# bcaitech1/p4-fr-sorry-math-but-love-you

Hardware: NVIDIA B200
Metric: EfficientSATRN greedy-decode images/sec (higher is better)
Workload: dtype bf16

## Files before the change

p4-fr-sorry-math-but-love-you_b200/csrc/kernels.h:

```cpp
#pragma once
#include "common.cuh"

namespace frx {

void launch_stem_conv(const float* in, const float* w, const float* scale, const float* shift, float* out,
                      int B, int Cin, int H, int W, int OH, int OW, int Cout, cudaStream_t st);
void launch_direct_conv3x3(const float* in, const float* w, const float* scale, const float* shift, float* out, int B,
                           int Cin, int H, int W, int OH, int OW, int Cout, int stride, int pad, int act,
                           cudaStream_t st);
void launch_igemm_f32(const GemmP& p, cudaStream_t st);
void launch_dwconv_f32(const DwP& p, cudaStream_t st);
void launch_se_gate_f32(const float* x, const float* w1, const float* b1, const float* w2, const float* b2,
                        float* gate, int B, int HW, int C, int R, cudaStream_t st);
void launch_maxpool2_f32(const float* in, float* out, int B, int H, int W, int C, cudaStream_t st);
void launch_pe2d_f32(const float* x, const float* w0, const float* b0, const float* w1, const float* b1,
                     const float* peh, const float* pew, float* out, int B, int h, int w, int C,
                     cudaStream_t st);
void launch_layernorm_f32(const float* x, const float* res, const float* gamma, const float* beta, float* out,
                          int M, int C, int scramble_S, cudaStream_t st);
void launch_enc_attn_f32(const float* qkv, float* out, int B, int S, int D, int heads, cudaStream_t st);
void launch_dec_gemm_f32(const DecGemmP& p, cudaStream_t st);
void launch_dec_attn_f32(const AttnP& p, int head_dim, cudaStream_t st);
void launch_fill_i32(int* p, int v, int n, cudaStream_t st);
void launch_dec_embed_f32(const int* tok, const long long* tok64, int fixed_token, const float* emb,
// ... 6 lines not shown


void launch_dec_sift_embed(float* logits, long long ld_logits, int V, long long* tokens_out, long long ld_tok, int4* state,
                           const int* flags, const int* limit, const SiftIds& ids, int* cur_tok, const float* emb,
                           const float* pe_next, float scale, float* x, int M, int D, cudaStream_t st);
void launch_sift_state_init(int4* state, int M, int sos, cudaStream_t st);
void launch_pad_mask(const long long* text, unsigned char* mask, int B, int L, int pad_id, cudaStream_t st);

void launch_swin_patch_embed(const float* img, const float* w, const float* bias, const float* g, const float* b,
                             const float* ape, float* out, int B, int IMGS, int R, int E, cudaStream_t st);
void launch_swin_window_attn(const float* qkv, const float* bias_table, float* out, int B, int R, int C, int heads, int ws,
                             int shift, cudaStream_t st);
bool launch_swin_window_attn_mma(const float* qkv, const float* bias_table, eh_t* out, int B, int R, int C, int heads,
                                 int ws, int shift, cudaStream_t st);
void launch_swin_patch_merge(const float* x, float* out, int B, int R, int C, cudaStream_t st);

void launch_beam_init(const BeamP& p, cudaStream_t st);
void launch_beam_select(const BeamP& p, cudaStream_t st);
void launch_beam_push(const BeamP& p, cudaStream_t st);
void launch_beam_finish(const BeamP& p, cudaStream_t st);

int launch_tc_igemm(TcGemmP p, cudaStream_t st);
int launch_tc_igemm_ws(TcGemmP p, int num_sms, cudaStream_t st);
void launch_pad_conv_weights(const eh_t* in, eh_t* out, long long rows, int Cin, cudaStream_t st);
void launch_h16_to_f32(const eh_t* in, float* out, long long n, cudaStream_t st);
void launch_f32_to_h16(const float* in, eh_t* out, long long n, cudaStream_t st);
void launch_stem_conv_bf16(const float* in, const float* w, const float* scale, const float* shift,
                           eh_t* out, int B, int Cin, int H, int W, int OH, int OW, int Cout, cudaStream_t st);
void launch_dwconv_bf16(const eh_t* in, const float* w, const float* scale, const float* shift,
                        eh_t* out, int B, int H, int W, int C, int OH, int OW, int stride, int pad_t,
                        int pad_l, int act, cudaStream_t st);
void launch_se_scale_bf16(eh_t* x, const float* w1, const float* b1, const float* w2, const float* b2,
                          int B, int HW, int C, int R, cudaStream_t st);
void launch_mbconv_dw_se_bf16(const eh_t* in, const float* w, const float* scale, const float* shift,
                              eh_t* out, float* mean, float* gate, const float* w1, const float* b1,
                              const float* w2, const float* b2, int B, int H, int W, int C, int OH, int OW, int stride,
                              int pad_t, int pad_l, int R, cudaStream_t st);
void launch_layernorm_bf16out(const float* x, const float* res, const float* gamma, const float* beta,
                              eh_t* out, int M, int C, int scramble_S, cudaStream_t st);
void launch_enc_attn_bf16out(const float* qkv, eh_t* out, int B, int S, int D, int heads, cudaStream_t st);
void launch_conv3x3_c24_bf16(const eh_t* in, const void* wfrag, const float* scale, const float* shift,
                             eh_t* out, int B, int H, int W, int add_res, cudaStream_t st);
void launch_lite_conv0_pool_bf16(const float* in, const float* w, const float* scale, const float* shift, eh_t* out,
                                 int B, int Cin, int H, int W, int Cout, cudaStream_t st);
void launch_maxpool2_bf16(const eh_t* in, eh_t* out, float* out_f32, int B, int H, int W, int C, cudaStream_t st);
bool launch_enc_attn_mma_bf16(const float* qkv, eh_t* out, int B, int S, int D, int heads, cudaStream_t st);
// ... 11 lines not shown
```

p4-fr-sorry-math-but-love-you_b200/csrc/kernels_tc.cu:

```cuda
#include <cuda.h>
#include <cuda_fp16.h>
#include <cudaTypedefs.h>

#include <cstdio>
#include <cstdlib>

#include "common.cuh"
#include "kernels.h"

namespace frx {

namespace {

constexpr int TC_BM = 128;
constexpr int TC_BK = 64;
constexpr int TC_STAGES = 3;
constexpr int TC_A_BYTES = TC_BM * TC_BK * 2;

__device__ __forceinline__ uint32_t smem_u32(const void* p) { return (uint32_t)__cvta_generic_to_shared(p); }

__device__ __forceinline__ void cp_async16(uint32_t dst, const void* src, uint32_t src_bytes) {
  asm volatile("cp.async.cg.shared.global [%0], [%1], 16, %2;\n" ::"r"(dst), "l"(src), "r"(src_bytes) : "memory");
}
__device__ __forceinline__ void cp_async_commit() { asm volatile("cp.async.commit_group;\n" ::: "memory"); }
// ... 14 lines not shown
__device__ __forceinline__ void tma_load_im2col(uint32_t smem_dst, const CUtensorMap* tmap, int c, int w, int h, int n,
                                                uint16_t w_off, uint16_t h_off, uint64_t* bar) {
  asm volatile(
      "cp.async.bulk.tensor.4d.shared::cluster.global.im2col.mbarrier::complete_tx::bytes [%0], [%1, {%3, %4, %5, %6}], [%2], {%7, %8};\n"
      ::"r"(smem_dst), "l"(reinterpret_cast<uint64_t>(tmap)), "r"(smem_u32(bar)), "r"(c), "r"(w), "r"(h), "r"(n),
        "h"(w_off), "h"(h_off) : "memory");
}
__device__ __forceinline__ void mbar_arrive(uint64_t* bar) {
  asm volatile("mbarrier.arrive.shared::cta.b64 _, [%0];\n" ::"r"(smem_u32(bar)) : "memory");
}
__device__ __forceinline__ void mbar_wait(uint64_t* bar, uint32_t parity) {
  const uint32_t addr = smem_u32(bar);
  uint32_t ok = 0;
  for (int spins = 0; spins < (1 << 24); ++spins) {
    asm volatile(
        "{\n"
        ".reg .pred p;\n"
        "mbarrier.try_wait.parity.shared::cta.b64 p, [%1], %2;\n"
        "selp.u32 %0, 1, 0, p;\n"
        "}\n" : "=r"(ok) : "r"(addr), "r"(parity) : "memory");
    if (ok) return;
  }
  __trap();
}

__device__ __forceinline__ uint64_t make_smem_desc(uint32_t saddr) {
  uint64_t d = 0;
  d |= (uint64_t)((saddr >> 4) & 0x3FFF);
  d |= (uint64_t)1 << 16;
  d |= (uint64_t)(1024 >> 4) << 32;
  d |= (uint64_t)1 << 46;
  d |= (uint64_t)2 << 61;
  return d;
}

__device__ __forceinline__ uint32_t make_idesc(int bn) {
  constexpr uint32_t fmt = FRX_ENC_FP16 ? 0u : 1u;
  return (1u << 4) | (fmt << 7) | (fmt << 10) | ((uint32_t)(bn >> 3) << 17) | ((uint32_t)(TC_BM >> 4) << 24);
}

__device__ __forceinline__ void umma_f16(uint32_t tmem_d, uint64_t adesc, uint64_t bdesc, uint32_t idesc, uint32_t accumulate) {
  asm volatile(
      "{\n"
      ".reg .pred p;\n"
      "setp.ne.b32 p, %4, 0;\n"
      "tcgen05.mma.cta_group::1.kind::f16 [%0], %1, %2, %3, p;\n"
// ... 60 lines not shown
        v[i + 1] = act_fast<ACT>(fmaf(v[i + 1], s.y, h.y));
        v[i + 2] = act_fast<ACT>(fmaf(v[i + 2], s.z, h.z));
        v[i + 3] = act_fast<ACT>(fmaf(v[i + 3], s.w, h.w));
      }
    }
  } else if (shift) {
#pragma unroll
    for (int i = 0; i < 16; i += 4) {
      const float4 h = __ldg(reinterpret_cast<const float4*>(shift + nb + i));
      v[i] = act_fast<ACT>(v[i] + h.x);
      v[i + 1] = act_fast<ACT>(v[i + 1] + h.y);
      v[i + 2] = act_fast<ACT>(v[i + 2] + h.z);
      v[i + 3] = act_fast<ACT>(v[i + 3] + h.w);
    }
  } else {
#pragma unroll
    for (int i = 0; i < 16; ++i) v[i] = act_fast<ACT>(v[i]);
  }
}

}

template <bool GELU>
__device__ __forceinline__ void epilogue_store16(const TcGemmP& p, const uint32_t (&r)[16], int m, int nb) {
      float v[16];
#pragma unroll
      for (int i = 0; i < 16; ++i) v[i] = __uint_as_float(r[i]);
      const bool full = nb + 16 <= p.N;
      if (full) {
        if (p.act == ACT_SILU) epi_affine_act<ACT_SILU>(v, p.scale, p.shift, nb);
        else if (p.act == ACT_RELU) epi_affine_act<ACT_RELU>(v, p.scale, p.shift, nb);
        else if (GELU && p.act == ACT_GELU) epi_affine_act<ACT_GELU>(v, p.scale, p.shift, nb);
        else epi_affine_act<ACT_NONE>(v, p.scale, p.shift, nb);
      } else {
#pragma unroll
        for (int i = 0; i < 16; ++i) {
          const int n = nb + i;
          if (n < p.N) {
            if (p.scale) v[i] = v[i] * __ldg(p.scale + n) + __ldg(p.shift + n);
            else if (p.shift) v[i] += __ldg(p.shift + n);
            v[i] = act_apply(v[i], p.act);
          }
        }
      }
      if (p.res) {
        if (p.res_f32) {
          const float* rp = reinterpret_cast<const float*>(p.res) + (size_t)m * p.ldr + nb;
          if (full) {
#pragma unroll
            for (int i = 0; i < 16; i += 4) {
              const float4 rr = __ldg(reinterpret_cast<const float4*>(rp + i));
              v[i] += rr.x; v[i + 1] += rr.y; v[i + 2] += rr.z; v[i + 3] += rr.w;
            }
          } else {
            for (int i = 0; i < 16; ++i)
              if (nb + i < p.N) v[i] += __ldg(rp + i);
          }
        } else {
          const eh_t* rp = reinterpret_cast<const eh_t*>(p.res) + (size_t)m * p.ldr + nb;
          if (full) {
            const uint4 r0 = __ldg(reinterpret_cast<const uint4*>(rp)), r1 = __ldg(reinterpret_cast<const uint4*>(rp + 8));
            const uint32_t rw[8] = {r0.x, r0.y, r0.z, r0.w, r1.x, r1.y, r1.z, r1.w};
#pragma unroll
            for (int i = 0; i < 8; ++i) {
              const float2 rf = eh2_unpack(rw[i]);
              v[2 * i] += rf.x;
              v[2 * i + 1] += rf.y;
            }
          } else {
            for (int i = 0; i < 16; ++i)
              if (nb + i < p.N) v[i] += eh_to_float(rp[i]);
          }
        }
      }
      if (p.out_f32) {
        float* cp = reinterpret_cast<float*>(p.C) + (size_t)m * p.ldc + nb;
        if (full && (p.ldc & 7) == 0 && (reinterpret_cast<uintptr_t>(p.C) & 31) == 0) {
#pragma unroll
          for (int i = 0; i < 16; i += 8)
            asm volatile("st.global.v8.f32 [%0], {%1, %2, %3, %4, %5, %6, %7, %8};\n" ::"l"(cp + i), "f"(v[i]), "f"(v[i + 1]),
                         "f"(v[i + 2]), "f"(v[i + 3]), "f"(v[i + 4]), "f"(v[i + 5]), "f"(v[i + 6]), "f"(v[i + 7]) : "memory");
        } else if (full && (p.ldc & 3) == 0) {
#pragma unroll
          for (int i = 0; i < 16; i += 4) *reinterpret_cast<float4*>(cp + i) = make_float4(v[i], v[i + 1], v[i + 2], v[i + 3]);
        } else {
// ... 160 lines not shown
      const int nb = n0 + cc * 16;
      if (m_ok && nb < p.N) epilogue_store16<false>(p, r, m, nb);
    }
  }
  tc_fence_before();
  __syncthreads();
  if (warp == 0) {
    asm volatile("tcgen05.dealloc.cta_group::1.sync.aligned.b32 %0, %1;\n" ::"r"(tmem), "n"(NCOLS) : "memory");
  }
}


constexpr int WS_STAGES = 4;
constexpr int WS_LAG = 2;
constexpr int WS_PROD_WARPS = 8;
constexpr int WS_EPI_WARPS = 8;
constexpr int WS_MMA_WARP = WS_PROD_WARPS + WS_EPI_WARPS;
constexpr int WS_TMA_WARP = WS_MMA_WARP + 1;
constexpr int WS_THREADS = (WS_TMA_WARP + 1) * 32;
constexpr int WS_PROD_THREADS = WS_PROD_WARPS * 32;
constexpr int WS_ROWS_PER_PASS = WS_PROD_THREADS / 8;
constexpr int WS_A_PASSES = TC_BM / WS_ROWS_PER_PASS;

template <int NCOLS, bool GELU>
__global__ void __launch_bounds__(WS_THREADS, NCOLS >= 256 ? 1 : 2) tc_igemm_ws_kernel(const TcGemmP p, const __grid_constant__ CUtensorMap tmA,
                                                                  const __grid_constant__ CUtensorMap tmW) {
  extern __shared__ unsigned char dyn_smem[];
  __shared__ __align__(8) uint64_t full_bar[WS_STAGES], empty_bar[WS_STAGES], acc_full[2], acc_empty[2];
  __shared__ uint32_t tmem_base_s;

  const int tid = threadIdx.x, warp = tid >> 5, lane = tid & 31;
  const int BN = p.BN;
  const uint32_t stage_bytes = TC_A_BYTES + (uint32_t)BN * (TC_BK * 2);
  const uint32_t smem0 = (smem_u32(dyn_smem) + 1023u) & ~1023u;
  const int KB = p.im2col ? p.KW * p.KW : (p.K + TC_BK - 1) / TC_BK;
  const int tiles_n = (p.N + BN - 1) / BN;
  const int tiles_m = (p.M + TC_BM - 1) / TC_BM;
  const int num_tiles = tiles_m * tiles_n;
  const bool gather = p.conv && !p.im2col;

  if (warp == WS_MMA_WARP) {
    asm volatile("tcgen05.alloc.cta_group::1.sync.aligned.shared::cta.b32 [%0], %1;\n" ::"r"(smem_u32(&tmem_base_s)), "n"(NCOLS) : "memory");
    asm volatile("tcgen05.relinquish_alloc_permit.cta_group::1.sync.aligned;\n" ::: "memory");
  }
  if (tid == 0) {
#pragma unroll
    for (int s = 0; s < WS_STAGES; ++s) { mbar_init(&full_bar[s], (gather ? WS_PROD_THREADS : 0) + 1); mbar_init(&empty_bar[s], 1); }
    mbar_init(&acc_full[0], 1); mbar_init(&acc_full[1], 1);
    const int epi_threads = (WS_EPI_WARPS + (gather ? 0 : WS_PROD_WARPS)) * 32;
    mbar_init(&acc_empty[0], epi_threads); mbar_init(&acc_empty[1], epi_threads);
    asm volatile("fence.mbarrier_init.release.cluster;\n" ::: "memory");
  }
  tc_fence_before();
  __syncthreads();
  tc_fence_after();
  const uint32_t tmem = tmem_base_s;

  if (gather ? warp < WS_PROD_WARPS : warp == WS_TMA_WARP) {
    const bool tma_thread = gather ? tid == 0 : lane == 0;
    const uint32_t tma_bytes = (uint32_t)BN * (TC_BK * 2) + (gather ? 0u : (uint32_t)TC_A_BYTES);
    if (!gather && !tma_thread) {
    } else {
    const int c = tid & 7, rbase = tid >> 3;
    int it = 0;
    for (int tile = blockIdx.x; tile < num_tiles; tile += gridDim.x) {
      const int m0 = (tile / tiles_n) * TC_BM, n0 = (tile % tiles_n) * BN;
      const eh_t* a_ptr[WS_A_PASSES];
      int a_ih0[WS_A_PASSES], a_iw0[WS_A_PASSES];
      bool a_ok[WS_A_PASSES];
      int bw = 0, bh = 0, bn = 0;
      if (p.im2col) {
        const int ow = m0 % p.OW, tq = m0 / p.OW;
        bw = ow * p.stride - p.pad_l;
        bh = (tq % p.OH) * p.stride - p.pad_t;
        bn = tq / p.OH;
      }
      if (gather) {
#pragma unroll
        for (int i = 0; i < WS_A_PASSES; ++i) {
          const int m = m0 + rbase + WS_ROWS_PER_PASS * i;
          a_ok[i] = m < p.M;
          a_ih0[i] = a_iw0[i] = 0;
          a_ptr[i] = p.A;
          if (a_ok[i]) {
            const int ow = m % p.OW;
            const int tq = m / p.OW;
            const int oh = tq % p.OH;
            const int n = tq / p.OH;
            a_ptr[i] = p.A + (size_t)n * p.H * p.Wd * p.Cin;
            a_ih0[i] = oh * p.stride - p.pad_t;
            a_iw0[i] = ow * p.stride - p.pad_l;
          }
        }
      }
      for (int kb = 0; kb < KB; ++kb, ++it) {
        const int stage = it % WS_STAGES;
        mbar_wait(&empty_bar[stage], (uint32_t)(((it / WS_STAGES) & 1) ^ 1));
        const uint32_t sa = smem0 + (uint32_t)stage * stage_bytes, sb = sa + TC_A_BYTES;
        if (tma_thread) {
          mbar_arrive_expect_tx(&full_bar[stage], tma_bytes);
          tma_load_2d(sb, &tmW, kb * TC_BK, n0, &full_bar[stage]);
          if (p.im2col) tma_load_im2col(sa, &tmA, 0, bw, bh, bn, (uint16_t)(kb % p.KW), (uint16_t)(kb / p.KW), &full_bar[stage]);
          else if (!p.conv) tma_load_2d(sa, &tmA, kb * TC_BK, m0, &full_bar[stage]);
        }
        if (gather) {
          const int k = kb * TC_BK + c * 8;
          const int tap = k / p.Cin;
          const int ci = k - tap * p.Cin;
          const int kh = tap / p.KW;
          const int kw = tap - kh * p.KW;
#pragma unroll
          for (int i = 0; i < WS_A_PASSES; ++i) {
            const int row = rbase + WS_ROWS_PER_PASS * i;
            const uint32_t dst = sa + (uint32_t)(row >> 3) * 1024u + (uint32_t)(row & 7) * 128u + (uint32_t)((c ^ (row & 7)) << 4);
            const eh_t* src = p.A;
            uint32_t bytes = 0;
            if (a_ok[i] && k < p.K) {
              const int ih = a_ih0[i] + kh, iw = a_iw0[i] + kw;
              if (ih >= 0 && ih < p.H && iw >= 0 && iw < p.Wd) {
                src = a_ptr[i] + ((size_t)ih * p.Wd + iw) * p.Cin + ci;
                bytes = 16;
              }
            }
            cp_async16(dst, src, bytes);
          }
          cp_async_commit();
          if (it >= WS_LAG) {
            cp_async_wait<WS_LAG>();
            asm volatile("fence.proxy.async.shared::cta;\n" ::: "memory");
            mbar_arrive(&full_bar[(it - WS_LAG) % WS_STAGES]);
          }
        }
      }
    }
    if (gather) {
      cp_async_wait<0>();
      asm volatile("fence.proxy.async.shared::cta;\n" ::: "memory");
      for (int j = (it >= WS_LAG ? it - WS_LAG : 0); j < it; ++j) mbar_arrive(&full_bar[j % WS_STAGES]);
    }
    }
  } else if (warp == WS_MMA_WARP) {
    if (lane == 0) {
      const uint32_t idesc = make_idesc(BN);
      int it = 0, ti = 0;
      for (int tile = blockIdx.x; tile < num_tiles; tile += gridDim.x, ++ti) {
        const int a = ti & 1;
        mbar_wait(&acc_empty[a], (uint32_t)(((ti >> 1) & 1) ^ 1));
        tc_fence_after();
        const uint32_t tacc = tmem + (uint32_t)(a * (NCOLS / 2));
        for (int kb = 0; kb < KB; ++kb, ++it) {
          const int stage = it % WS_STAGES;
          mbar_wait(&full_bar[stage], (uint32_t)((it / WS_STAGES) & 1));
          tc_fence_after();
          const uint32_t sa = smem0 + (uint32_t)stage * stage_bytes;
          const uint64_t adesc = make_smem_desc(sa), bdesc = make_smem_desc(sa + TC_A_BYTES);
#pragma unroll
          for (int j = 0; j < TC_BK / 16; ++j)
            umma_f16(tacc, adesc + (uint64_t)(2 * j), bdesc + (uint64_t)(2 * j), idesc, (kb | j) ? 1u : 0u);
          umma_commit(&empty_bar[stage]);
          if (kb == KB - 1) umma_commit(&acc_full[a]);
        }
      }
    }
  } else if (warp < WS_MMA_WARP) {
    const int q = warp & 3;
    const int nsub = (WS_EPI_WARPS + (gather ? 0 : WS_PROD_WARPS)) / 4;
    const int sub = (gather ? warp - WS_PROD_WARPS : warp) >> 2;
    int ti = 0;
    for (int tile = blockIdx.x; tile < num_tiles; tile += gridDim.x, ++ti) {
      const int a = ti & 1;
      const int m0 = (tile / tiles_n) * TC_BM, n0 = (tile % tiles_n) * BN;
      mbar_wait(&acc_full[a], (uint32_t)((ti >> 1) & 1));
      tc_fence_after();
      const int m = m0 + q * 32 + lane;
      const bool m_ok = m < p.M;
      const uint32_t tacc = tmem + (uint32_t)(a * (NCOLS / 2)) + ((uint32_t)(q * 32) << 16);
      for (int cc = sub; cc * 16 < BN; cc += nsub) {
        uint32_t r[16];
        tmem_ld16(tacc + (uint32_t)(cc * 16), r);
        const int nb = n0 + cc * 16;
        if (m_ok && nb < p.N) epilogue_store16<GELU>(p, r, m, nb);
      }
      tc_fence_before();
      mbar_arrive(&acc_empty[a]);
    }
  }
  tc_fence_before();
  __syncthreads();
  if (warp == WS_MMA_WARP) {
    asm volatile("tcgen05.dealloc.cta_group::1.sync.aligned.b32 %0, %1;\n" ::"r"(tmem), "n"(NCOLS) : "memory");
  }
}

static int tc_pick_bn(int N) {
  if (N <= 256) return (N + 15) / 16 * 16;
  for (int bn = 256; bn >= 128; bn -= 16)
    if (N % bn == 0) return bn;
  return 256;
}

template <int NCOLS>
static int tc_launch(const TcGemmP& p, cudaStream_t st) {
  const size_t smem = (size_t)p.stages * (TC_A_BYTES + (size_t)p.BN * TC_BK * 2) + 1024;
  static SmemOptIn opt;
  {
    cudaError_t e = opt.ensure(tc_igemm_kernel<NCOLS>, smem, true);
    if (e != cudaSuccess) return (int)e;
  }
// ... 35 lines not shown
    if (cudaGetDriverEntryPoint("cuTensorMapEncodeIm2col", &ptr, cudaEnableDefault, &qres) == cudaSuccess &&
        qres == cudaDriverEntryPointSuccess)
      fn = reinterpret_cast<PFN_cuTensorMapEncodeIm2col_v12000>(ptr);
  }
  return fn;
}

static int make_tmap_im2col(CUtensorMap* tm, const TcGemmP& p) {
  PFN_cuTensorMapEncodeIm2col_v12000 enc = im2col_map_encoder();
  if (!enc) return (int)cudaErrorNotSupported;
  const int B = p.M / (p.OH * p.OW), k = p.KW;
  const int pad_r = (p.OW - 1) * p.stride + k - p.Wd - p.pad_l, pad_b = (p.OH - 1) * p.stride + k - p.H - p.pad_t;
  cuuint64_t dims[4] = {(cuuint64_t)p.Cin, (cuuint64_t)p.Wd, (cuuint64_t)p.H, (cuuint64_t)B};
  cuuint64_t strides[3] = {(cuuint64_t)p.Cin * 2, (cuuint64_t)p.Wd * p.Cin * 2, (cuuint64_t)p.H * p.Wd * p.Cin * 2};
  int lower[2] = {-p.pad_l, -p.pad_t};
  int upper[2] = {pad_r - (k - 1), pad_b - (k - 1)};
  cuuint32_t estr[4] = {1, (cuuint32_t)p.stride, (cuuint32_t)p.stride, 1};
  CUresult r = enc(tm, (FRX_ENC_FP16 ? CU_TENSOR_MAP_DATA_TYPE_FLOAT16 : CU_TENSOR_MAP_DATA_TYPE_BFLOAT16), 4, const_cast<eh_t*>(p.A), dims, strides, lower, upper,
                   (cuuint32_t)TC_BK, (cuuint32_t)TC_BM, estr, CU_TENSOR_MAP_INTERLEAVE_NONE, CU_TENSOR_MAP_SWIZZLE_128B,
                   CU_TENSOR_MAP_L2_PROMOTION_L2_128B, CU_TENSOR_MAP_FLOAT_OOB_FILL_NONE);
  return r == CUDA_SUCCESS ? 0 : (int)cudaErrorInvalidValue;
}

template <int NCOLS>
static int tc_launch_ws(const TcGemmP& p_in, int num_sms, cudaStream_t st) {
  TcGemmP p = p_in;
  const size_t smem = (size_t)WS_STAGES * (TC_A_BYTES + (size_t)p.BN * TC_BK * 2) + 1024;
  static SmemOptIn opt, opt_gelu;
  {
    cudaError_t e = opt.ensure(tc_igemm_ws_kernel<NCOLS, false>, smem, true);
    if (e == cudaSuccess) e = opt_gelu.ensure(tc_igemm_ws_kernel<NCOLS, true>, smem, true);
    if (e != cudaSuccess) return (int)e;
  }
  const int tiles = ((p.M + TC_BM - 1) / TC_BM) * ((p.N + p.BN - 1) / p.BN);
  int per_sm = (int)((227 * 1024) / (smem + 2048));
  if (per_sm > 512 / NCOLS) per_sm = 512 / NCOLS;
  if (per_sm > 4) per_sm = 4;
  if (per_sm < 1) per_sm = 1;
  const int grid = tiles < num_sms * per_sm ? tiles : num_sms * per_sm;
  CUtensorMap tmA, tmW;
  int rc;
  p.im2col = 0;
  if (p.conv && p.Wpad && p.Cin <= TC_BK && p.M % (p.OH * p.OW) == 0 && make_tmap_im2col(&tmA, p) == 0) {
    p.im2col = 1;
    rc = make_tmap_2d(&tmW, p.Wpad, p.N, (long long)p.KW * p.KW * TC_BK, (long long)p.KW * p.KW * TC_BK, p.BN);
  } else {
    rc = make_tmap_2d(&tmW, p.W, p.N, p.K, p.ldw, p.BN);
    if (rc) return rc;
    if (!p.conv) rc = make_tmap_2d(&tmA, p.A, p.M, p.K, p.lda, TC_BM);
    else tmA = tmW;
  }
  if (rc) return rc;
  if (getenv("FRX_DEBUG"))
    fprintf(stderr, "[frx] tc gemm M=%d N=%d K=%d BN=%d conv=%d Cin=%d stride=%d -> %s, grid %d\n", p.M, p.N, p.K, p.BN, p.conv,
            p.Cin, p.stride, p.im2col ? "TMA im2col" : (p.conv ? "cp.async gather" : "TMA dense"), grid);
  if (p.act == ACT_GELU) tc_igemm_ws_kernel<NCOLS, true><<<grid, WS_THREADS, smem, st>>>(p, tmA, tmW);
  else tc_igemm_ws_kernel<NCOLS, false><<<grid, WS_THREADS, smem, st>>>(p, tmA, tmW);
  return 0;
}

int launch_tc_igemm_ws(TcGemmP p, int num_sms, cudaStream_t st) {
  if (p.BN == 0) {
    p.BN = tc_pick_bn(p.N);
    const int tiles_m = (p.M + TC_BM - 1) / TC_BM;
    while (p.BN > 64 && p.BN % 32 == 0 && p.N % (p.BN / 2) == 0 && tiles_m * ((p.N + p.BN - 1) / p.BN) < num_sms) p.BN /= 2;
  }
  if (p.BN <= 32) { p.BN = 32; return tc_launch_ws<64>(p, num_sms, st); }
  if (p.BN <= 64) return tc_launch_ws<128>(p, num_sms, st);
  if (p.BN <= 128) return tc_launch_ws<256>(p, num_sms, st);
  return tc_launch_ws<512>(p, num_sms, st);
}

int launch_tc_igemm(TcGemmP p, cudaStream_t st) {
  if (p.act == ACT_GELU) {
    int dev = 0, sms = 148;
    cudaGetDevice(&dev);
    cudaDeviceGetAttribute(&sms, cudaDevAttrMultiProcessorCount, dev);
    return launch_tc_igemm_ws(p, sms, st);
  }
  if (p.BN == 0) p.BN = tc_pick_bn(p.N);
  {
    const int kb = (p.K + TC_BK - 1) / TC_BK;
    const size_t stage = TC_A_BYTES + (size_t)p.BN * TC_BK * 2;
    p.stages = (kb > 3 && 3 * stage <= 72 * 1024) ? 3 : 2;
  }
  if (p.BN <= 32) { p.BN = 32; return tc_launch<32>(p, st); }
  if (p.BN <= 64) return tc_launch<64>(p, st);
  if (p.BN <= 128) return tc_launch<128>(p, st);
  return tc_launch<256>(p, st);
}

__global__ void __launch_bounds__(256) f32_to_h16_kernel(const float* __restrict__ in, eh_t* __restrict__ out, long long n) {
  long long i = ((long long)blockIdx.x * blockDim.x + threadIdx.x) * 4;
// ... 35 lines not shown
```

p4-fr-sorry-math-but-love-you_b200/csrc/runtime.cu:

```cuda
#include <cmath>
#include <cstdarg>
#include <cstdio>
#include <cstring>
#include <map>
#include <string>
#include <vector>

#include "../../include/frx.h"
#include "kernels.h"
#include "runtime.h"

using namespace frx;

static int fail(frx_handle* h, const char* fmt, ...) {
  char buf[1024];
  va_list ap;
  va_start(ap, fmt);
  vsnprintf(buf, sizeof buf, fmt, ap);
  va_end(ap);
  if (h) h->err = buf;
  return 1;
}

#define CK(expr)                                                                          \
// ... 193 lines not shown
    return fail(h, "frx_load_tensor('%s'): unsupported dtype %d", name, dtype);
  }
  h->raw[name] = std::move(t);
  h->finalized = false;
  return 0;
}

extern "C" int frx_set_option(frx_handle* h, const char* key, int64_t value) {
  if (!h || !key) return 1;
  ON_DEVICE(h->cfg.device);
  std::string k(key);
  if (k == "taps") h->opt_taps = value != 0;
  else if (k == "graphs") h->opt_graphs = value != 0;
  else if (k == "step16") h->opt_step16 = value != 0;
  else if (k == "pipe_enc") h->opt_pipe_enc = value != 0;
  else if (k == "timing") h->opt_timing = value != 0;
  else if (k == "cluster_images") {}
  else if (k == "dec_hpc") h->opt_dec_hpc = (value == 1 || value == 2) ? (int)value : 0;
  else if (k == "conv24") h->opt_conv24 = value != 0;
  else if (k == "enc_fp32") h->opt_enc_fp32 = value != 0;
  else if (k == "tc_ws") h->opt_tc_ws = value != 0;
  else if (k == "train_splitk") h->opt_train_splitk = value != 0;
  else if (k == "tc_im2col") h->opt_tc_im2col = value != 0;
  else if (k == "prof") {
    h->opt_prof = value != 0;
    if (h->opt_prof && !h->prof) { void* p; if (dev_alloc(h, &p, 16 * 8)) return 1; h->prof = (long long*)p; }
  }
  else if (k == "parts") {
    if (h->ws_ready && ((int)value & 3) != h->opt_parts)
      return fail(h, "option 'parts' cannot change after the first frx_finalize_weights (create a new handle)");
    h->opt_parts = (int)value & 3;
    h->finalized = false;
  }
  else return fail(h, "unknown option '%s'", key);
  return 0;
}

extern "C" int64_t frx_launch_count(const frx_handle* h) { return h ? h->launches : 0; }
extern "C" int64_t frx_device_bytes(const frx_handle* h) { return h ? h->device_bytes : 0; }

extern "C" int frx_read_prof(frx_handle* h, int64_t* out16) {
  if (!h || !out16 || !h->prof) return fail(h, "profiling not enabled (frx_set_option(h, \"prof\", 1))");
  ON_DEVICE(h->cfg.device);
  CK(cudaMemcpy(out16, h->prof, 16 * 8, cudaMemcpyDeviceToHost));
  return 0;
}
// ... 777 lines not shown
  bf* x = (bf*)h->act[0];
  bf* y = (bf*)h->act[1];
  bf* m0 = (bf*)h->mid[0];
  bf* m1 = (bf*)h->mid[1];
  launch_stem_conv_bf16(images, A + h->stem_w, A + h->stem_sc, A + h->stem_sh, x, B, c.in_ch, c.height, c.width, H, W, 24, st);
  CKL();
  if (tap_bf16(h, "stem", x, B, H, W, 24, st)) return 1;
  for (const BlockW& b : h->blocks) {
    int OH, OW;
    if (b.kind == 0 && b.w_frag24 && h->opt_conv24) {
      OH = H; OW = W;
      launch_conv3x3_c24_bf16(x, A + b.w_frag24, A + b.sc_a, A + b.sh_a, y, B, H, W, b.residual ? 1 : 0, st);
      CKL();
    } else if (b.kind == 0) {
      TcGemmP g = tc_conv(x, B, H, W, b.cin, A, b.wb_a, b.cout, b.k, b.stride, y, &OH, &OW);
      if (b.wb_a_pad && h->opt_tc_im2col) g.Wpad = (const eh_t*)(A + b.wb_a_pad);
      g.scale = A + b.sc_a; g.shift = A + b.sh_a; g.act = ACT_SILU;
      if (b.residual) { g.res = x; g.ldr = b.cout; }
      TCL(g);
    } else if (b.kind == 1) {
      TcGemmP g = tc_conv(x, B, H, W, b.cin, A, b.wb_a, b.mid, b.k, b.stride, m0, &OH, &OW);
      if (b.wb_a_pad && h->opt_tc_im2col) g.Wpad = (const eh_t*)(A + b.wb_a_pad);
      g.scale = A + b.sc_a; g.shift = A + b.sh_a; g.act = ACT_SILU;
      TCL(g);
      TcGemmP g2 = tc_dense(m0, B * OH * OW, b.mid, A, b.wb_b, b.cout, y, 0);
      g2.scale = A + b.sc_b; g2.shift = A + b.sh_b;
      if (b.residual) { g2.res = x; g2.ldr = b.cout; }
      TCL(g2);
    } else {
      TcGemmP g = tc_dense(x, B * H * W, b.cin, A, b.wb_a, b.mid, m0, 0);
      g.scale = A + b.sc_a; g.shift = A + b.sh_a; g.act = ACT_SILU;
      TCL(g);
      int pt, pl;
      same_pad(H, b.k, b.stride, &OH, &pt);
      same_pad(W, b.k, b.stride, &OW, &pl);
      launch_mbconv_dw_se_bf16(m0, A + b.w_dw, A + b.sc_dw, A + b.sh_dw, m1, h->gate, h->gate + (size_t)B * 2048,
                               A + b.se_w1, A + b.se_b1, A + b.se_w2t, A + b.se_b2, B, H, W, b.mid, OH, OW, b.stride, pt, pl,
                               b.se_r, st);
      CKL(); h->launches += 2;
      TcGemmP g2 = tc_dense(m1, B * OH * OW, b.mid, A, b.wb_b, b.cout, y, 0);
      g2.scale = A + b.sc_b; g2.shift = A + b.sh_b;
      if (b.residual) { g2.res = x; g2.ldr = b.cout; }
      TCL(g2);
    }
    H = OH; W = OW;
    bf* t = x; x = y; y = t;
    if (tap_bf16(h, b.name, x, B, H, W, b.cout, st)) return 1;
  }
  if (H != h->feat_h || W != h->feat_w) return fail(h, "trunk output %dx%d != expected %dx%d", H, W, h->feat_h, h->feat_w);
  const int fh = h->feat_h, fw = h->feat_w, S = fh * fw, C = c.enc_hidden, F = c.enc_filter, M = B * S;
  float* tf = (float*)y;
// ... 849 lines not shown
```

p4-fr-sorry-math-but-love-you_b200/csrc/runtime.h:

```cpp
#pragma once
#include <cuda_runtime.h>
#include <stdint.h>

#include <map>
#include <string>
#include <tuple>
#include <vector>

#include "../../include/frx.h"

struct HostTensor {
  std::vector<int64_t> shape;
  std::vector<float> f;
};

struct BlockW {
  int kind;
  int cin, cout, k, stride, mid, se_r;
  bool residual;
  std::string name;
  size_t w_a, sc_a, sh_a;
  size_t w_dw, sc_dw, sh_dw;
  size_t se_w1, se_b1, se_w2, se_b2, se_w2t = 0;
  size_t w_b, sc_b, sh_b;
// ... 30 lines not shown
  double *hscore = nullptr, *nlogp = nullptr;
  int *hnode = nullptr, *nprev = nullptr, *ntok = nullptr, *nlen = nullptr, *nkv = nullptr, *chain = nullptr, *small = nullptr;
  float* logits = nullptr;
  int* host_flag = nullptr;
};
struct TfWs {
  float *x = nullptr, *y = nullptr, *z = nullptr, *qkv = nullptr, *ff = nullptr;
  unsigned char* mask = nullptr;
  void *xb = nullptr, *ffb = nullptr;
};

struct frx_handle {
  frx_config cfg{};
  std::string err;
  int num_sms = 0;
  std::map<std::string, HostTensor> raw;
  bool finalized = false, ws_ready = false;
  bool opt_taps = false, opt_graphs = true, opt_timing = false, opt_step16 = true, opt_pipe_enc = true;
  int* step_hist = nullptr;
  bool opt_prof = false;
  bool opt_tc_im2col = true;
  void* hook_wpad = nullptr; size_t hook_wpad_bytes = 0;
  bool opt_tc_ws = true;
  int opt_dec_hpc = 0;
  bool opt_conv24 = true;
  bool opt_enc_fp32 = false;
  long long* prof = nullptr;
  int opt_parts = 3;
  int feat_h = 0, feat_w = 0;
  std::vector<void*> allocs;
  int64_t device_bytes = 0, launches = 0;

  float* arena = nullptr;
  size_t arena_bytes = 0;
  size_t stem_w = 0, stem_sc = 0, stem_sh = 0, last_w = 0, last_sc = 0, last_sh = 0;
  std::vector<BlockW> blocks;
  LiteConvW lite[4]{};
  size_t pe_w0 = 0, pe_b0 = 0, pe_w1 = 0, pe_b1 = 0, pe_h = 0, pe_w = 0;
  std::vector<EncLayerW> enc;
  size_t sw_pe_w = 0, sw_pe_b = 0, sw_pe_g = 0, sw_pe_beta = 0, sw_ape = 0, sw_norm_g = 0, sw_norm_b = 0;
  std::vector<SwinBlockW> sw_blocks;
  std::vector<SwinMergeW> sw_merges;
  float *sw_x[2] = {nullptr, nullptr}, *sw_a = nullptr, *sw_qkv = nullptr, *sw_hid = nullptr;
  size_t emb = 0, pe1d = 0, gen_w = 0, gen_b = 0, w_cross = 0, b_cross = 0;
  size_t gen_wb = 0;
  size_t last_wb = 0, cross_wb = 0;
// ... 44 lines not shown
```

Measured before the change: 13030.

## Fuse fused-MBConv expansion conv and 1x1 projection into one warp-specialized tcgen05 kernel

Adds a FUSE variant of the warp-specialized tensor-core implicit GEMM. The conv's SiLU-activated output tile is written as bf16 into swizzled shared memory and then multiplied by the projection weights, which stay resident in shared memory, with residual add in the same kernel. The MMA warp interleaves projection MMAs with the next tile's conv MMAs by polling barriers. This removes the intermediate activation round trip through global memory and one kernel launch per fused-MBConv block. In exchange the smem ring shrinks, the grid covers only M tiles, and the barrier polling adds complexity.

Result: no change. 13040, median of 6 (+0.1%).

```diff
diff --git a/p4-fr-sorry-math-but-love-you_b200/csrc/kernels.h b/p4-fr-sorry-math-but-love-you_b200/csrc/kernels.h
--- a/p4-fr-sorry-math-but-love-you_b200/csrc/kernels.h
+++ b/p4-fr-sorry-math-but-love-you_b200/csrc/kernels.h
@@ -52,6 +52,7 @@
 
 int launch_tc_igemm(TcGemmP p, cudaStream_t st);
 int launch_tc_igemm_ws(TcGemmP p, int num_sms, cudaStream_t st);
+int launch_tc_conv_proj_ws(TcGemmP p, TcGemmP p2, int num_sms, cudaStream_t st);
 void launch_pad_conv_weights(const eh_t* in, eh_t* out, long long rows, int Cin, cudaStream_t st);
 void launch_h16_to_f32(const eh_t* in, float* out, long long n, cudaStream_t st);
 void launch_f32_to_h16(const float* in, eh_t* out, long long n, cudaStream_t st);
diff --git a/p4-fr-sorry-math-but-love-you_b200/csrc/kernels_tc.cu b/p4-fr-sorry-math-but-love-you_b200/csrc/kernels_tc.cu
--- a/p4-fr-sorry-math-but-love-you_b200/csrc/kernels_tc.cu
+++ b/p4-fr-sorry-math-but-love-you_b200/csrc/kernels_tc.cu
@@ -60,6 +60,17 @@
     if (ok) return;
   }
   __trap();
+}
+
+__device__ __forceinline__ bool mbar_test(uint64_t* bar, uint32_t parity) {
+  uint32_t ok;
+  asm volatile(
+      "{\n"
+      ".reg .pred p;\n"
+      "mbarrier.test_wait.parity.shared::cta.b64 p, [%1], %2;\n"
+      "selp.u32 %0, 1, 0, p;\n"
+      "}\n" : "=r"(ok) : "r"(smem_u32(bar)), "r"(parity) : "memory");
+  return ok != 0;
 }
 
 __device__ __forceinline__ uint64_t make_smem_desc(uint32_t saddr) {
@@ -166,7 +177,8 @@
 }
 
 template <bool GELU>
-__device__ __forceinline__ void epilogue_store16(const TcGemmP& p, const uint32_t (&r)[16], int m, int nb) {
+__device__ __forceinline__ void epilogue_store16(const TcGemmP& p, const uint32_t (&r)[16], int m, int nb,
+                                                 const uint32_t* res_pre = nullptr) {
       float v[16];
 #pragma unroll
       for (int i = 0; i < 16; ++i) v[i] = __uint_as_float(r[i]);
@@ -203,8 +215,14 @@
         } else {
           const eh_t* rp = reinterpret_cast<const eh_t*>(p.res) + (size_t)m * p.ldr + nb;
           if (full) {
-            const uint4 r0 = __ldg(reinterpret_cast<const uint4*>(rp)), r1 = __ldg(reinterpret_cast<const uint4*>(rp + 8));
-            const uint32_t rw[8] = {r0.x, r0.y, r0.z, r0.w, r1.x, r1.y, r1.z, r1.w};
+            uint32_t rw[8];
+            if (res_pre) {
+#pragma unroll
+              for (int i = 0; i < 8; ++i) rw[i] = res_pre[i];
+            } else {
+              const uint4 r0 = __ldg(reinterpret_cast<const uint4*>(rp)), r1 = __ldg(reinterpret_cast<const uint4*>(rp + 8));
+              rw[0] = r0.x; rw[1] = r0.y; rw[2] = r0.z; rw[3] = r0.w; rw[4] = r1.x; rw[5] = r1.y; rw[6] = r1.z; rw[7] = r1.w;
+            }
 #pragma unroll
             for (int i = 0; i < 8; ++i) {
               const float2 rf = eh2_unpack(rw[i]);
@@ -411,17 +429,24 @@
 constexpr int WS_ROWS_PER_PASS = WS_PROD_THREADS / 8;
 constexpr int WS_A_PASSES = TC_BM / WS_ROWS_PER_PASS;
 
-template <int NCOLS, bool GELU>
+template <int NCOLS, bool GELU, bool FUSE>
 __global__ void __launch_bounds__(WS_THREADS, NCOLS >= 256 ? 1 : 2) tc_igemm_ws_kernel(const TcGemmP p, const __grid_constant__ CUtensorMap tmA,
-                                                                  const __grid_constant__ CUtensorMap tmW) {
+                                                                  const __grid_constant__ CUtensorMap tmW, const TcGemmP p2,
+                                                                  const __grid_constant__ CUtensorMap tmW2) {
   extern __shared__ unsigned char dyn_smem[];
   __shared__ __align__(8) uint64_t full_bar[WS_STAGES], empty_bar[WS_STAGES], acc_full[2], acc_empty[2];
+  __shared__ __align__(8) uint64_t w2_full, e_full, proj_full;
   __shared__ uint32_t tmem_base_s;
 
   const int tid = threadIdx.x, warp = tid >> 5, lane = tid & 31;
   const int BN = p.BN;
+  const int NS = FUSE ? p.stages : WS_STAGES;
   const uint32_t stage_bytes = TC_A_BYTES + (uint32_t)BN * (TC_BK * 2);
   const uint32_t smem0 = (smem_u32(dyn_smem) + 1023u) & ~1023u;
+  const int KB2 = FUSE ? (BN + TC_BK - 1) / TC_BK : 0;
+  const uint32_t e_smem = smem0 + (uint32_t)NS * stage_bytes;
+  const uint32_t w2_smem = e_smem + (uint32_t)KB2 * TC_A_BYTES;
+  const uint32_t w2_slab = (uint32_t)p2.BN * (TC_BK * 2);
   const int KB = p.im2col ? p.KW * p.KW : (p.K + TC_BK - 1) / TC_BK;
   const int tiles_n = (p.N + BN - 1) / BN;
   const int tiles_m = (p.M + TC_BM - 1) / TC_BM;
@@ -438,6 +463,7 @@
     mbar_init(&acc_full[0], 1); mbar_init(&acc_full[1], 1);
     const int epi_threads = (WS_EPI_WARPS + (gather ? 0 : WS_PROD_WARPS)) * 32;
     mbar_init(&acc_empty[0], epi_threads); mbar_init(&acc_empty[1], epi_threads);
+    if (FUSE) { mbar_init(&w2_full, 1); mbar_init(&e_full, epi_threads); mbar_init(&proj_full, 1); }
     asm volatile("fence.mbarrier_init.release.cluster;\n" ::: "memory");
   }
   tc_fence_before();
@@ -451,6 +477,10 @@
     if (!gather && !tma_thread) {
     } else {
     const int c = tid & 7, rbase = tid >> 3;
+    if (FUSE && tma_thread) {
+      mbar_arrive_expect_tx(&w2_full, (uint32_t)KB2 * w2_slab);
+      for (int kb = 0; kb < KB2; ++kb) tma_load_2d(w2_smem + (uint32_t)kb * w2_slab, &tmW2, kb * TC_BK, 0, &w2_full);
+    }
     int it = 0;
     for (int tile = blockIdx.x; tile < num_tiles; tile += gridDim.x) {
       const int m0 = (tile / tiles_n) * TC_BM, n0 = (tile % tiles_n) * BN;
@@ -483,8 +513,8 @@
         }
       }
       for (int kb = 0; kb < KB; ++kb, ++it) {
-        const int stage = it % WS_STAGES;
-        mbar_wait(&empty_bar[stage], (uint32_t)(((it / WS_STAGES) & 1) ^ 1));
+        const int stage = it % NS;
+        mbar_wait(&empty_bar[stage], (uint32_t)(((it / NS) & 1) ^ 1));
         const uint32_t sa = smem0 + (uint32_t)stage * stage_bytes, sb = sa + TC_A_BYTES;
         if (tma_thread) {
           mbar_arrive_expect_tx(&full_bar[stage], tma_bytes);
@@ -517,7 +547,7 @@
           if (it >= WS_LAG) {
             cp_async_wait<WS_LAG>();
             asm volatile("fence.proxy.async.shared::cta;\n" ::: "memory");
-            mbar_arrive(&full_bar[(it - WS_LAG) % WS_STAGES]);
+            mbar_arrive(&full_bar[(it - WS_LAG) % NS]);
           }
         }
       }
@@ -525,21 +555,43 @@
     if (gather) {
       cp_async_wait<0>();
       asm volatile("fence.proxy.async.shared::cta;\n" ::: "memory");
-      for (int j = (it >= WS_LAG ? it - WS_LAG : 0); j < it; ++j) mbar_arrive(&full_bar[j % WS_STAGES]);
+      for (int j = (it >= WS_LAG ? it - WS_LAG : 0); j < it; ++j) mbar_arrive(&full_bar[j % NS]);
     }
     }
   } else if (warp == WS_MMA_WARP) {
     if (lane == 0) {
       const uint32_t idesc = make_idesc(BN);
+      auto projection = [&](int t) {
+        if (t == 0) mbar_wait(&w2_full, 0);
+        mbar_wait(&e_full, (uint32_t)(t & 1));
+        tc_fence_after();
+        const uint32_t idesc2 = make_idesc(p2.BN), tacc = tmem + (uint32_t)((t & 1) * (NCOLS / 2));
+        for (int kb = 0; kb < KB2; ++kb) {
+          const uint64_t adesc = make_smem_desc(e_smem + (uint32_t)kb * TC_A_BYTES), bdesc = make_smem_desc(w2_smem + (uint32_t)kb * w2_slab);
+#pragma unroll
+          for (int j = 0; j < TC_BK / 16; ++j)
+            umma_f16(tacc, adesc + (uint64_t)(2 * j), bdesc + (uint64_t)(2 * j), idesc2, (kb | j) ? 1u : 0u);
+        }
+        umma_commit(&proj_full);
+      };
+      int pend = -1;
+      auto wait = [&](uint64_t* bar, uint32_t parity) {
+        if (!FUSE) { mbar_wait(bar, parity); return; }
+        for (int spins = 0; !mbar_test(bar, parity); ++spins) {
+          if (pend >= 0 && mbar_test(&e_full, (uint32_t)(pend & 1))) { projection(pend); pend = -1; }
+          if (spins == (1 << 24)) __trap();
+        }
+      };
       int it = 0, ti = 0;
       for (int tile = blockIdx.x; tile < num_tiles; tile += gridDim.x, ++ti) {
         const int a = ti & 1;
-        mbar_wait(&acc_empty[a], (uint32_t)(((ti >> 1) & 1) ^ 1));
+        wait(&acc_empty[a], (uint32_t)(((ti >> 1) & 1) ^ 1));
         tc_fence_after();
         const uint32_t tacc = tmem + (uint32_t)(a * (NCOLS / 2));
         for (int kb = 0; kb < KB; ++kb, ++it) {
-          const int stage = it % WS_STAGES;
-          mbar_wait(&full_bar[stage], (uint32_t)((it / WS_STAGES) & 1));
+          const int stage = it % NS;
+          if (FUSE && pend >= 0 && mbar_test(&e_full, (uint32_t)(pend & 1))) { projection(pend); pend = -1; }
+          wait(&full_bar[stage], (uint32_t)((it / NS) & 1));
           tc_fence_after();
           const uint32_t sa = smem0 + (uint32_t)stage * stage_bytes;
           const uint64_t adesc = make_smem_desc(sa), bdesc = make_smem_desc(sa + TC_A_BYTES);
@@ -549,12 +601,67 @@
           umma_commit(&empty_bar[stage]);
           if (kb == KB - 1) umma_commit(&acc_full[a]);
         }
-      }
+        if (FUSE) {
+          if (pend >= 0) projection(pend);
+          pend = ti;
+        }
+      }
+      if (FUSE && pend >= 0) projection(pend);
     }
   } else if (warp < WS_MMA_WARP) {
     const int q = warp & 3;
     const int nsub = (WS_EPI_WARPS + (gather ? 0 : WS_PROD_WARPS)) / 4;
     const int sub = (gather ? warp - WS_PROD_WARPS : warp) >> 2;
+    if (FUSE) {
+      const int row = q * 32 + lane;
+      const uint32_t erow = e_smem + (uint32_t)(row >> 3) * 1024u + (uint32_t)(row & 7) * 128u;
+      int ti = 0;
+      for (int tile = blockIdx.x; tile < num_tiles; tile += gridDim.x, ++ti) {
+        const int a = ti & 1;
+        const int m = tile * TC_BM + row;
+        const bool out_ok = m < p2.M && sub * 16 < p2.N;
+        uint32_t rw[8];
+        if (out_ok && p2.res) {
+          const uint4* rp = reinterpret_cast<const uint4*>(reinterpret_cast<const eh_t*>(p2.res) + (size_t)m * p2.ldr + sub * 16);
+          const uint4 r0 = __ldg(rp), r1 = __ldg(rp + 1);
+          rw[0] = r0.x; rw[1] = r0.y; rw[2] = r0.z; rw[3] = r0.w; rw[4] = r1.x; rw[5] = r1.y; rw[6] = r1.z; rw[7] = r1.w;
+        }
+        mbar_wait(&acc_full[a], (uint32_t)((ti >> 1) & 1));
+        tc_fence_after();
+        const uint32_t tacc = tmem + (uint32_t)(a * (NCOLS / 2)) + ((uint32_t)(q * 32) << 16);
+        for (int cc = sub; cc * 16 < KB2 * TC_BK; cc += 4) {
+          uint32_t w[8] = {0u, 0u, 0u, 0u, 0u, 0u, 0u, 0u};
+          if (cc * 16 < BN) {
+            uint32_t r[16];
+            tmem_ld16(tacc + (uint32_t)(cc * 16), r);
+            float v[16];
+#pragma unroll
+            for (int i = 0; i < 16; ++i) v[i] = __uint_as_float(r[i]);
+            epi_affine_act<ACT_SILU>(v, p.scale, p.shift, cc * 16);
+#pragma unroll
+            for (int i = 0; i < 8; ++i) w[i] = eh2_pack(v[2 * i], v[2 * i + 1]);
+          }
+          const uint32_t slab = erow + (uint32_t)(cc >> 2) * TC_A_BYTES;
+          const int c0 = (cc & 3) * 2;
+          asm volatile("st.shared.v4.b32 [%0], {%1, %2, %3, %4};\n" ::"r"(slab + (uint32_t)((c0 ^ (row & 7)) << 4)),
+                       "r"(w[0]), "r"(w[1]), "r"(w[2]), "r"(w[3]) : "memory");
+          asm volatile("st.shared.v4.b32 [%0], {%1, %2, %3, %4};\n" ::"r"(slab + (uint32_t)(((c0 + 1) ^ (row & 7)) << 4)),
+                       "r"(w[4]), "r"(w[5]), "r"(w[6]), "r"(w[7]) : "memory");
+        }
+        asm volatile("fence.proxy.async.shared::cta;\n" ::: "memory");
+        tc_fence_before();
+        mbar_arrive(&e_full);
+        mbar_wait(&proj_full, (uint32_t)(ti & 1));
+        tc_fence_after();
+        if (sub * 16 < p2.BN) {
+          uint32_t r[16];
+          tmem_ld16(tacc + (uint32_t)(sub * 16), r);
+          if (out_ok) epilogue_store16<false>(p2, r, m, sub * 16, rw);
+        }
+        tc_fence_before();
+        mbar_arrive(&acc_empty[a]);
+      }
+    } else {
     int ti = 0;
     for (int tile = blockIdx.x; tile < num_tiles; tile += gridDim.x, ++ti) {
       const int a = ti & 1;
@@ -573,6 +680,7 @@
       tc_fence_before();
       mbar_arrive(&acc_empty[a]);
     }
+    }
   }
   tc_fence_before();
   __syncthreads();
@@ -654,14 +762,25 @@
   return r == CUDA_SUCCESS ? 0 : (int)cudaErrorInvalidValue;
 }
 
+static int make_conv_tmaps(TcGemmP& p, CUtensorMap* tmA, CUtensorMap* tmW) {
+  p.im2col = 0;
+  if (p.Wpad && p.Cin <= TC_BK && p.M % (p.OH * p.OW) == 0 && make_tmap_im2col(tmA, p) == 0) {
+    p.im2col = 1;
+    return make_tmap_2d(tmW, p.Wpad, p.N, (long long)p.KW * p.KW * TC_BK, (long long)p.KW * p.KW * TC_BK, p.BN);
+  }
+  const int rc = make_tmap_2d(tmW, p.W, p.N, p.K, p.ldw, p.BN);
+  *tmA = *tmW;
+  return rc;
+}
+
 template <int NCOLS>
 static int tc_launch_ws(const TcGemmP& p_in, int num_sms, cudaStream_t st) {
   TcGemmP p = p_in;
   const size_t smem = (size_t)WS_STAGES * (TC_A_BYTES + (size_t)p.BN * TC_BK * 2) + 1024;
   static SmemOptIn opt, opt_gelu;
   {
-    cudaError_t e = opt.ensure(tc_igemm_ws_kernel<NCOLS, false>, smem, true);
-    if (e == cudaSuccess) e = opt_gelu.ensure(tc_igemm_ws_kernel<NCOLS, true>, smem, true);
+    cudaError_t e = opt.ensure(tc_igemm_ws_kernel<NCOLS, false, false>, smem, true);
+    if (e == cudaSuccess) e = opt_gelu.ensure(tc_igemm_ws_kernel<NCOLS, true, false>, smem, true);
     if (e != cudaSuccess) return (int)e;
   }
   const int tiles = ((p.M + TC_BM - 1) / TC_BM) * ((p.N + p.BN - 1) / p.BN);
@@ -673,21 +792,49 @@
   CUtensorMap tmA, tmW;
   int rc;
   p.im2col = 0;
-  if (p.conv && p.Wpad && p.Cin <= TC_BK && p.M % (p.OH * p.OW) == 0 && make_tmap_im2col(&tmA, p) == 0) {
-    p.im2col = 1;
-    rc = make_tmap_2d(&tmW, p.Wpad, p.N, (long long)p.KW * p.KW * TC_BK, (long long)p.KW * p.KW * TC_BK, p.BN);
+  if (p.conv) {
+    rc = make_conv_tmaps(p, &tmA, &tmW);
   } else {
     rc = make_tmap_2d(&tmW, p.W, p.N, p.K, p.ldw, p.BN);
     if (rc) return rc;
-    if (!p.conv) rc = make_tmap_2d(&tmA, p.A, p.M, p.K, p.lda, TC_BM);
-    else tmA = tmW;
+    rc = make_tmap_2d(&tmA, p.A, p.M, p.K, p.lda, TC_BM);
   }
   if (rc) return rc;
   if (getenv("FRX_DEBUG"))
     fprintf(stderr, "[frx] tc gemm M=%d N=%d K=%d BN=%d conv=%d Cin=%d stride=%d -> %s, grid %d\n", p.M, p.N, p.K, p.BN, p.conv,
             p.Cin, p.stride, p.im2col ? "TMA im2col" : (p.conv ? "cp.async gather" : "TMA dense"), grid);
-  if (p.act == ACT_GELU) tc_igemm_ws_kernel<NCOLS, true><<<grid, WS_THREADS, smem, st>>>(p, tmA, tmW);
-  else tc_igemm_ws_kernel<NCOLS, false><<<grid, WS_THREADS, smem, st>>>(p, tmA, tmW);
+  if (p.act == ACT_GELU) tc_igemm_ws_kernel<NCOLS, true, false><<<grid, WS_THREADS, smem, st>>>(p, tmA, tmW, p, tmW);
+  else tc_igemm_ws_kernel<NCOLS, false, false><<<grid, WS_THREADS, smem, st>>>(p, tmA, tmW, p, tmW);
+  return 0;
+}
+
+template <int NCOLS>
+static int tc_launch_ws_proj(const TcGemmP& p_in, const TcGemmP& p2, int num_sms, cudaStream_t st) {
+  TcGemmP p = p_in;
+  const size_t stage = TC_A_BYTES + (size_t)p.BN * TC_BK * 2;
+  const int kb2 = (p.BN + TC_BK - 1) / TC_BK;
+  const size_t fixed = (size_t)kb2 * (TC_A_BYTES + (size_t)p2.BN * TC_BK * 2) + 1024;
+  const size_t budget = 227 * 1024 - 1024;
+  if (fixed + 2 * stage > budget) return (int)cudaErrorInvalidValue;
+  p.stages = (int)((budget - fixed) / stage);
+  if (p.stages > WS_STAGES) p.stages = WS_STAGES;
+  const size_t smem = fixed + (size_t)p.stages * stage;
+  static SmemOptIn opt;
+  {
+    cudaError_t e = opt.ensure(tc_igemm_ws_kernel<NCOLS, false, true>, smem, true);
+    if (e != cudaSuccess) return (int)e;
+  }
+  const int tiles = (p.M + TC_BM - 1) / TC_BM;
+  const int grid = tiles < num_sms ? tiles : num_sms;
+  CUtensorMap tmA, tmW, tmW2;
+  int rc = make_conv_tmaps(p, &tmA, &tmW);
+  if (rc == 0) rc = make_tmap_2d(&tmW2, p2.W, p2.N, p2.K, p2.ldw, p2.BN);
+  if (rc) return rc;
+  if (!p.im2col) return (int)cudaErrorInvalidValue;
+  if (getenv("FRX_DEBUG"))
+    fprintf(stderr, "[frx] tc conv+projection M=%d N=%d K=%d BN=%d Cin=%d stride=%d, N2=%d BN2=%d, ring %d, grid %d\n", p.M,
+            p.N, p.K, p.BN, p.Cin, p.stride, p2.N, p2.BN, p.stages, grid);
+  tc_igemm_ws_kernel<NCOLS, false, true><<<grid, WS_THREADS, smem, st>>>(p, tmA, tmW, p2, tmW2);
   return 0;
 }
 
@@ -701,6 +848,16 @@
   if (p.BN <= 64) return tc_launch_ws<128>(p, num_sms, st);
   if (p.BN <= 128) return tc_launch_ws<256>(p, num_sms, st);
   return tc_launch_ws<512>(p, num_sms, st);
+}
+
+int launch_tc_conv_proj_ws(TcGemmP p, TcGemmP p2, int num_sms, cudaStream_t st) {
+  p.BN = (p.N + 15) / 16 * 16;
+  p2.BN = tc_pick_bn(p2.N);
+  if (!p.conv || p.res || p.act != ACT_SILU || !p.scale || p.N % 16 || p.N > 256 || p2.conv || p2.K != p.N ||
+      p2.M != p.M || p2.BN > 64)
+    return (int)cudaErrorInvalidValue;
+  if (p.BN <= 128) return tc_launch_ws_proj<256>(p, p2, num_sms, st);
+  return tc_launch_ws_proj<512>(p, p2, num_sms, st);
 }
 
 int launch_tc_igemm(TcGemmP p, cudaStream_t st) {
diff --git a/p4-fr-sorry-math-but-love-you_b200/csrc/runtime.cu b/p4-fr-sorry-math-but-love-you_b200/csrc/runtime.cu
--- a/p4-fr-sorry-math-but-love-you_b200/csrc/runtime.cu
+++ b/p4-fr-sorry-math-but-love-you_b200/csrc/runtime.cu
@@ -239,6 +239,7 @@
   else if (k == "tc_ws") h->opt_tc_ws = value != 0;
   else if (k == "train_splitk") h->opt_train_splitk = value != 0;
   else if (k == "tc_im2col") h->opt_tc_im2col = value != 0;
+  else if (k == "enc_fuse") h->opt_enc_fuse = value != 0;
   else if (k == "prof") {
     h->opt_prof = value != 0;
     if (h->opt_prof && !h->prof) { void* p; if (dev_alloc(h, &p, 16 * 8)) return 1; h->prof = (long long*)p; }
@@ -1062,11 +1063,17 @@
       TcGemmP g = tc_conv(x, B, H, W, b.cin, A, b.wb_a, b.mid, b.k, b.stride, m0, &OH, &OW);
       if (b.wb_a_pad && h->opt_tc_im2col) g.Wpad = (const eh_t*)(A + b.wb_a_pad);
       g.scale = A + b.sc_a; g.shift = A + b.sh_a; g.act = ACT_SILU;
-      TCL(g);
       TcGemmP g2 = tc_dense(m0, B * OH * OW, b.mid, A, b.wb_b, b.cout, y, 0);
       g2.scale = A + b.sc_b; g2.shift = A + b.sh_b;
       if (b.residual) { g2.res = x; g2.ldr = b.cout; }
-      TCL(g2);
+      if (h->opt_enc_fuse && h->opt_tc_ws && g.Wpad) {
+        const int rc = launch_tc_conv_proj_ws(g, g2, h->num_sms, st);
+        if (rc) return fail(h, "fused conv + projection configuration failed: %s", cudaGetErrorString((cudaError_t)rc));
+        CKL();
+      } else {
+        TCL(g);
+        TCL(g2);
+      }
     } else {
       TcGemmP g = tc_dense(x, B * H * W, b.cin, A, b.wb_a, b.mid, m0, 0);
       g.scale = A + b.sc_a; g.shift = A + b.sh_a; g.act = ACT_SILU;
diff --git a/p4-fr-sorry-math-but-love-you_b200/csrc/runtime.h b/p4-fr-sorry-math-but-love-you_b200/csrc/runtime.h
--- a/p4-fr-sorry-math-but-love-you_b200/csrc/runtime.h
+++ b/p4-fr-sorry-math-but-love-you_b200/csrc/runtime.h
@@ -76,6 +76,7 @@
   bool opt_tc_im2col = true;
   void* hook_wpad = nullptr; size_t hook_wpad_bytes = 0;
   bool opt_tc_ws = true;
+  bool opt_enc_fuse = true;
   int opt_dec_hpc = 0;
   bool opt_conv24 = true;
   bool opt_enc_fp32 = false;
```
